# menezesandre/stackrl

Hardware: AMD Instinct MI355X
Metric: env steps/sec (batched Stack-v0) (higher is better)
Workload: dtype f32

## Files before the change

### include/stackrl_qnet.h

```cpp
#ifndef STACKRL_QNET_H_
#define STACKRL_QNET_H_

#include <stdint.h>

#ifdef __cplusplus
extern "C" {
#endif

int srl_xcorr_forward(const float* x_dev, const float* w_dev, float* out_dev, int32_t B, int32_t C, int32_t H,
                      int32_t W, int32_t kh, int32_t kw, void* stream);

int64_t srl_xcorr_mfma_scratch_bytes(int32_t mode, int32_t precision, int32_t B, int32_t C, int32_t H, int32_t kh);
int srl_xcorr_mfma(int32_t mode, int32_t precision, const void* in_dev, int32_t in_f32, const void* kern_dev,
                   int32_t kern_f32, float* out_dev, void* scratch_dev, int64_t scratch_bytes, int32_t B, int32_t C,
                   int32_t H, int32_t kh, void* stream);
const char* srl_xcorr_mfma_last_error(void);

int srl_bias_act(const void* in_dev, void* out_dev, const float* bias_dev, int64_t npix, int32_t C, int32_t out_stride,
                 int32_t out_offset, int32_t nchw_hw, int32_t relu, void* stream);
int srl_bias_act_pool(const void* in_dev, void* skip_dev, void* pooled_dev, const float* bias_dev, int32_t B, int32_t H,
                      int32_t W, int32_t C, int32_t skip_stride, int32_t skip_offset, void* stream);
int srl_bias_act_f32(const float* in_dev, float* out_dev, const float* bias_dev, int64_t npix, int32_t C,
                     int32_t out_stride, int32_t out_offset, int32_t nchw_hw, int32_t relu, void* stream);
int srl_bias_act_pool_f32(const float* in_dev, float* skip_dev, float* pooled_dev, const float* bias_dev, int32_t B,
// ... 57 lines not shown

int srl_baseline_select(const double* values_dev, const uint8_t* mask_dev, int32_t use_goal, int32_t minorder,
                        int64_t* actions_dev, double* neg_values_dev, int32_t B, int32_t OH, void* stream);

const char* srl_qnet_last_error(void);
const char* srl_qnet_build_info(void);

int srl_td_epilogue(const float* q_dev, const float* q_next_online_dev, const float* q_next_target_dev,
                    const int64_t* actions_dev, const float* rewards_dev, const uint8_t* terminal_dev,
                    const float* weights_dev, float gamma, float huber_delta, float reward_scale, int32_t use_double,
                    float prio_eps, int32_t mb, int32_t A, float* loss_dev, float* mean_td_dev, float* td_abs_dev,
                    float* logits_dev, float* grad_q_dev, float* scratch_dev, int32_t* ticket_dev, void* stream);

int srl_adam_step(float* params_dev, const float* grads_dev, float* m_dev, float* v_dev, int64_t n, float* state_dev,
                  float lr, float beta1, float beta2, float eps, void* stream);

int64_t srl_gumbel_topk_scratch_bytes(int64_t n, int32_t k);
int srl_gumbel_topk(const float* logits_dev, const float* u_dev, const float* alpha_dev, int64_t n, int32_t k,
                    int64_t* out_idx_dev, float* out_key_dev, void* scratch_dev, int64_t scratch_bytes, void* stream);

int srl_replay_scatter(const uint8_t* state0_dev, const uint8_t* state1_dev, int64_t bytes0, int64_t bytes1,
                       const float* reward_dev, const uint8_t* terminal_dev, const int64_t* action_dev, int32_t B,
                       int64_t slot, int64_t part_len, uint8_t* mem0_dev, uint8_t* mem1_dev, float* mem_reward_dev,
                       uint8_t* mem_terminal_dev, int64_t* mem_action_dev, float* mem_logits_dev, void* stream);
int srl_replay_gather(const int64_t* idx_dev, int32_t mb, int64_t part_len, int64_t n_steps, int32_t literal_next,
                      int64_t* next_dev, const uint8_t* mem0_dev, const uint8_t* mem1_dev, int64_t bytes0, int64_t bytes1,
                      const float* mem_reward_dev, const uint8_t* mem_terminal_dev, const int64_t* mem_action_dev,
                      const float* mem_logits_dev, const float* alpha_dev, const float* beta_dev,
                      const float* min_logit_dev, uint8_t* state0_dev, uint8_t* state1_dev, uint8_t* next0_dev,
                      uint8_t* next1_dev, int64_t* action_dev, float* reward_dev, uint8_t* terminal_dev,
                      float* weight_dev, void* stream);
int64_t srl_logit_extrema_scratch_bytes(void);
int srl_logit_extrema(const float* logits_dev, int64_t n, float* out_v2_dev, int64_t* out_i2_dev, void* scratch_dev, void* stream);
const char* srl_learner_last_error(void);

int srl_tconv(const float* x_dev, int32_t x_stride, int32_t x_off, const float* wp_dev, const float* bias_dev, float* y_dev,
              int32_t y_stride, int32_t y_off, int32_t B, int32_t H, int32_t W, int32_t cin, int32_t cout, int32_t taps,
              int32_t relu, int32_t d2s, void* stream);
int64_t srl_twrw_scratch_floats(int32_t B, int32_t H, int32_t W, int32_t cin, int32_t cout, int32_t taps);
int srl_twrw(const float* x_dev, int32_t x_stride, int32_t x_off, const float* gz_dev, float* gw_dev, float* scratch_dev,
             int32_t B, int32_t H, int32_t W, int32_t cin, int32_t cout, int32_t taps, int32_t convt,
             const float* bias_partial_dev, int32_t bias_nblk, int32_t bias_C, float* gbias_dev, void* stream);
int64_t srl_tact_bwd_scratch_floats(int64_t npix, int32_t C);
int32_t srl_tact_bwd_blocks(int64_t npix, int32_t C);
int srl_tact_bwd(const float* g_dev, int32_t g_stride, int32_t g_off, const float* y_dev, int32_t y_stride, int32_t y_off,
                 const float* gpool_dev, float* gz_dev, float* gbias_dev, float* scratch_dev, int32_t B, int32_t H, int32_t W,
                 int32_t C, int32_t relu, int32_t s2d, void* stream);
int srl_trepack(const float* flat_dev, float* packed_dev, const int64_t* desc_dev, int32_t nlayers, int64_t total, void* stream);
int srl_thead_fwd(const float* z_dev, const float* pw_dev, const float* pb_dev, const float* v_dev, float* q_dev, int32_t B,
                  int32_t A, void* stream);
int srl_thead_bwd(const float* z_dev, const float* pw_dev, const float* gq_dev, float* gz_dev, float* gv_dev, float* gpw_dev,
                  float* gpb_dev, float* scratch_dev, int32_t n, int32_t A, void* stream);
int srl_tvalue_fwd(const float* x0_dev, const float* W1_dev, const float* b1_dev, const float* W2_dev, const float* b2_dev,
                   float* pooled_dev, float* h_dev, float* v_dev, int32_t B, int32_t P, int32_t C, int32_t U, void* stream);
int srl_tvalue_bwd(const float* gv_dev, const float* h_dev, const float* pooled_dev, const float* W1_dev, const float* W2_dev,
                   const float* gin_dev, float* gx_dev, float* gW1_dev, float* gb1_dev, float* gW2_dev, float* gb2_dev,
                   float* scratch_dev, int32_t n, int32_t P, int32_t C, int32_t U, void* stream);
int srl_tlayout(const float* src_dev, int32_t src_stride, int32_t src_off, float* dst_dev, int32_t B, int32_t HW, int32_t C,
                int32_t to_nhwc, void* stream);
int srl_tcorr_grad(const float* g_dev, int32_t g_stride, float* plain_dev, float* padded_dev, int32_t n, int32_t O, int32_t pad,
                   void* stream);
int srl_tflip(const float* in_dev, float* out_dev, int64_t planes, int32_t hw, void* stream);
int srl_tu8_to_f32(const uint8_t* in_dev, float* out_dev, int64_t n, void* stream);
const char* srl_train_conv_last_error(void);

#ifdef __cplusplus
// ... 4 lines not shown
```

### stackrl_amd/csrc/learner.hip

```cpp
#include <hip/hip_runtime.h>
#include <stdint.h>
#include <math.h>
#include "../../include/stackrl_qnet.h"

namespace {

thread_local char g_err[256] = "";
int fail(const char* m) { snprintf(g_err, sizeof g_err, "%s", m); return 1; }
#define HIPCHK(x) do { hipError_t e_ = (x); if (e_ != hipSuccess) return fail(hipGetErrorString(e_)); } while (0)

__device__ __forceinline__ uint32_t f2o(float f) {
  const uint32_t u = __float_as_uint(f);
  return u ^ ((uint32_t)((int32_t)u >> 31) | 0x80000000u);
}
__device__ __forceinline__ uint64_t vkey(float v, uint32_t idx) { return ((uint64_t)f2o(v) << 32) | (uint32_t)(~idx); }

__device__ __forceinline__ uint64_t wave_max_u64(uint64_t k) {
#pragma unroll
  for (int s = 32; s >= 1; s >>= 1) {
    const uint32_t lo = __shfl_xor((uint32_t)k, s), hi = __shfl_xor((uint32_t)(k >> 32), s);
    const uint64_t o = ((uint64_t)hi << 32) | lo;
    k = o > k ? o : k;
  }
  return k;
}

template <int T>
__device__ __forceinline__ uint64_t block_max_u64(uint64_t k, uint64_t* sh) {
  k = wave_max_u64(k);
  const int w = threadIdx.x >> 6;
  __syncthreads();
  if ((threadIdx.x & 63) == 0) sh[w] = k;
  __syncthreads();
  uint64_t r = sh[0];
#pragma unroll
  for (int i = 1; i < T / 64; ++i) r = sh[i] > r ? sh[i] : r;
// ... 208 lines not shown
__device__ __forceinline__ void ext_take(Ext& a, const Ext& b) {
  if (b.mx > a.mx || (b.mx == a.mx && b.imx < a.imx)) { a.mx = b.mx; a.imx = b.imx; }
  if (b.mn < a.mn || (b.mn == a.mn && b.imn < a.imn)) { a.mn = b.mn; a.imn = b.imn; }
}
__device__ __forceinline__ Ext ext_block(Ext e, Ext* sh) {
  sh[threadIdx.x] = e;
  __syncthreads();
  for (int s = 128; s >= 1; s >>= 1) {
    if ((int)threadIdx.x < s) { Ext a = sh[threadIdx.x]; ext_take(a, sh[threadIdx.x + s]); sh[threadIdx.x] = a; }
    __syncthreads();
  }
  return sh[0];
}
__global__ void __launch_bounds__(256) k_logit_extrema(const float* __restrict__ logits, long long n, Ext* __restrict__ part) {
  __shared__ Ext sh[256];
  Ext e; e.mx = -INFINITY; e.imx = 0x7fffffffffffffffLL; e.mn = INFINITY; e.imn = 0x7fffffffffffffffLL;
  for (long long i = (long long)blockIdx.x * 256 + threadIdx.x; i < n; i += (long long)gridDim.x * 256) {
    const float v = logits[i];
    Ext o; o.mx = v; o.imx = i; o.mn = (v - v == 0.0f) ? v : INFINITY; o.imn = i;
    ext_take(e, o);
  }
  const Ext r = ext_block(e, sh);
  if (threadIdx.x == 0) part[blockIdx.x] = r;
}
__global__ void __launch_bounds__(256) k_logit_extrema_finish(const Ext* __restrict__ part, int nblk, float* __restrict__ out_v,
                                                              long long* __restrict__ out_i) {
  __shared__ Ext sh[256];
  Ext e; e.mx = -INFINITY; e.imx = 0x7fffffffffffffffLL; e.mn = INFINITY; e.imn = 0x7fffffffffffffffLL;
  if ((int)threadIdx.x < nblk) e = part[threadIdx.x];
  const Ext r = ext_block(e, sh);
  if (threadIdx.x == 0) { out_v[0] = r.mx; out_i[0] = r.imx; out_v[1] = r.mn; out_i[1] = r.imn; }
}

}

extern "C" {

const char* srl_learner_last_error(void) { return g_err; }

int srl_td_epilogue(const float* q, const float* qn_online, const float* qn_target, const int64_t* actions,
                    const float* rewards, const uint8_t* terminal, const float* weights, float gamma, float huber_delta,
                    float reward_scale, int32_t use_double, float prio_eps, int32_t mb, int32_t A, float* out_loss,
                    float* out_mtd, float* td_abs, float* logits, float* grad_q, float* scratch, int32_t* ticket,
                    void* stream) {
  if (!q || !qn_target || (use_double && !qn_online) || !actions || !rewards || !terminal || !out_loss || !out_mtd ||
      !td_abs || !logits || !scratch || !ticket || mb < 1 || A < 1)
    return fail("srl_td_epilogue: bad argument");
  hipLaunchKernelGGL((k_td_epilogue<256>), dim3(mb), dim3(256), 0, (hipStream_t)stream, q, qn_online, qn_target, actions,
                     rewards, terminal, weights, gamma, huber_delta, reward_scale, (int)use_double, prio_eps, (int)mb, (int)A,
                     out_loss, out_mtd, td_abs, logits, grad_q, scratch, (int*)ticket);
  HIPCHK(hipGetLastError());
  return 0;
}

int srl_adam_step(float* params, const float* grads, float* m, float* v, int64_t n, float* state, float lr, float beta1,
                  float beta2, float eps, void* stream) {
  if (!params || !grads || !m || !v || !state || n < 1) return fail("srl_adam_step: bad argument");
  if (((uintptr_t)params | (uintptr_t)grads | (uintptr_t)m | (uintptr_t)v) & 15) return fail("srl_adam_step: buffers must be 16-byte aligned");
  hipLaunchKernelGGL(k_adam_tick, dim3(1), dim3(64), 0, (hipStream_t)stream, state, lr, beta1, beta2);
  const int64_t groups = (n >> 2) + 1;
  hipLaunchKernelGGL(k_adam_step, dim3((unsigned)((groups + 255) / 256)), dim3(256), 0, (hipStream_t)stream, params, grads, m,
                     v, n, (const float*)state, beta1, beta2, eps);
  HIPCHK(hipGetLastError());
  return 0;
}

int64_t srl_gumbel_topk_scratch_bytes(int64_t n, int32_t k) {
  if (n < 1 || k < 1) return -1;
  const int64_t G = (n + SRL_TOPK_CHUNK - 1) / SRL_TOPK_CHUNK;
  return G * k * (int64_t)(sizeof(float) + sizeof(int32_t));
}
// ... 28 lines not shown
  return 0;
}

int srl_replay_gather(const int64_t* idx, int32_t mb, int64_t part_len, int64_t n_steps, int32_t literal_next, int64_t* o_next,
                      const uint8_t* m0, const uint8_t* m1, int64_t bytes0,
                      int64_t bytes1, const float* m_reward, const uint8_t* m_terminal, const int64_t* m_action,
                      const float* m_logits, const float* alpha, const float* beta, const float* min_logit, uint8_t* o_s0,
                      uint8_t* o_s1, uint8_t* o_n0, uint8_t* o_n1, int64_t* o_action, float* o_reward, uint8_t* o_terminal,
                      float* o_weight, void* stream) {
  if (!idx || part_len < 1 || n_steps < 1 || !m0 || !m1 || !m_reward || !m_terminal || !m_action || !m_logits || !o_s0 || !o_s1 || !o_n0 || !o_n1 ||
      !o_action || !o_reward || !o_terminal || mb < 1 || (bytes0 & 15) || (bytes1 & 15) || (o_weight && (!alpha || !beta || !min_logit)))
    return fail("srl_replay_gather: bad argument (rows must be multiples of 16 bytes)");
  const int64_t vec = 2 * ((bytes0 + bytes1) >> 4);
  const unsigned gx = (unsigned)((vec + 255) / 256 > 32 ? 32 : (vec + 255) / 256);
  hipLaunchKernelGGL(k_replay_gather, dim3(gx, mb), dim3(256), 0, (hipStream_t)stream, idx, part_len, n_steps, (int)literal_next, o_next, m0, m1, bytes0, bytes1, m_reward,
                     m_terminal, m_action, m_logits, alpha, beta, min_logit, o_s0, o_s1, o_n0, o_n1, o_action, o_reward, o_terminal,
                     o_weight);
  HIPCHK(hipGetLastError());
  return 0;
}

int64_t srl_logit_extrema_scratch_bytes(void) { return 256 * (int64_t)sizeof(Ext); }

int srl_logit_extrema(const float* logits, int64_t n, float* out_v2, int64_t* out_i2, void* scratch, void* stream) {
  if (!logits || n < 1 || !out_v2 || !out_i2 || !scratch) return fail("srl_logit_extrema: bad argument");
  const int nblk = (int)((n + 1023) / 1024 > 256 ? 256 : (n + 1023) / 1024);
  hipStream_t st = (hipStream_t)stream;
  hipLaunchKernelGGL(k_logit_extrema, dim3(nblk), dim3(256), 0, st, logits, (long long)n, (Ext*)scratch);
  hipLaunchKernelGGL(k_logit_extrema_finish, dim3(1), dim3(256), 0, st, (const Ext*)scratch, nblk, out_v2, (long long*)out_i2);
  HIPCHK(hipGetLastError());
  return 0;
}

}
```

### stackrl_amd/dqn.py

```python
import math

import torch
import torch.distributed as dist

from stackrl_amd.memory import ReplayMemory


CAPTURE_MODE = 'thread_local'


class PolynomialDecay(object):

  def __init__(self, initial_learning_rate, decay_steps, end_learning_rate=0.0001, power=1.0):
    self.initial, self.steps, self.end, self.power = float(initial_learning_rate), int(decay_steps), float(end_learning_rate), float(power)

  def __call__(self, step):
    s = min(int(step), self.steps)
    return (self.initial - self.end) * (1 - s / self.steps) ** self.power + self.end


EXPLORATION_MODES = ['epsilon-greedy', 'boltzmann']


def philox4x32_10(counter, key):
# ... 376 lines not shown
      linear = td_abs - quadratic
      loss = 0.5 * quadratic ** 2 + self._huber_delta * linear
    else:
      loss = 0.5 * td_abs ** 2
    if weights is not None:
      loss = loss * weights
    return loss.mean()

  def _draw(self):
    if self._prioritized:
      indexes, weights, (states, actions, rewards, next_states, terminal) = \
        self._replay_memory.sample(self._minibatch_size, get_weights=True)
    else:
      indexes = weights = None
      states, actions, rewards, next_states, terminal = self._replay_memory.sample(self._minibatch_size)
    return (indexes, weights) + tuple(states) + (actions, rewards) + tuple(next_states) + (terminal,)

  def _next_minibatch(self):
    k = self._prefetch
    if not k:
      flat = self._draw()
    else:
      flat = self._peek_minibatch()
      self._advance_fifo()
    return self._split_minibatch(flat)

  def _peek_minibatch(self):
    if self._fifo is None:
      self._fifo = [tuple(None if t is None else t.clone() for t in self._draw()) for _ in range(self._prefetch)]
    return tuple(None if t is None else t.clone() for t in self._fifo[0])

  def _advance_fifo(self):
    k = self._prefetch
    for i in range(k - 1):
      for dst, src in zip(self._fifo[i], self._fifo[i + 1]):
        if dst is not None:
          dst.copy_(src)
    for dst, src in zip(self._fifo[k - 1], self._draw()):
      if dst is not None:
        dst.copy_(src)

  @staticmethod
  def _split_minibatch(flat):
    indexes, weights = flat[0], flat[1]
    ns = (len(flat) - 5) // 2
    states, actions, rewards = flat[2:2 + ns], flat[2 + ns], flat[3 + ns]
    next_states, terminal = flat[4 + ns:4 + 2 * ns], flat[4 + 2 * ns]
    return indexes, weights, (states, actions, rewards, next_states, terminal)

  def _forward_backward(self, peek=False):
    indexes, weights, (states, actions, rewards, next_states, terminal) = \
      self._split_minibatch(self._peek_minibatch()) if peek else self._next_minibatch()
    if not self._bias_compensation:
      weights = None
    self._last_sample_indexes = indexes
    new_logits = None
    if self._fused and not (self._gamma == 0 and not self._n_step):
      from stackrl_amd import qops
      if self._hand is not None:
        mb = int(actions.shape[0])
        self._hand.refresh()
        with torch.no_grad():
          tq = self._hand_t.forward(next_states)
          if self._n_step:
            rewards = (self._gamma_r * rewards).sum(dim=-1)
        if self._double:
          both = tuple(torch.cat([a, b]) for a, b in zip(states, next_states))
          q2 = self._hand.forward(both, save=True)
          q_all, qo = q2[:mb], q2[mb:].detach()
        else:
          q_all, qo = self._hand.forward(states, save=True), None
# ... 232 lines not shown
```

### stackrl_amd/memory.py

```python
import math

import torch


class ReplayMemory(object):
  def __init__(self, state_spec, max_length, alpha=None, beta=None, iters_counter=None, n_steps=None,
               epsilon=1e-3, seed=None, device=None, reference_next_index=True):
    self.device = torch.device(device) if device is not None else torch.device('cpu')
    self._n_parts = int(state_spec[0][0][0])
    max_length -= max_length % self._n_parts
    self._max_length = max_length // self._n_parts
    self._size = max_length
    self._offsets = torch.arange(self._n_parts, dtype=torch.int64, device=self.device) * self._max_length
    if (callable(alpha) or callable(beta)) and iters_counter is None:
      raise ValueError('iters_counter must be provided with a callable alpha/beta')
    self._alpha = alpha if callable(alpha) else float(alpha or 0.)
    self._beta = beta if callable(beta) else float(1. if beta is None else beta)
    self._iters_counter = iters_counter
    self._n_steps = int(n_steps or 1)
    self._n_range = torch.arange(1, self._n_steps + 1, dtype=torch.int64, device=self.device)
    assert self._max_length > self._n_steps
    if epsilon <= 0:
      raise ValueError('epsilon must be greater than 0')
    self.epsilon = float(epsilon)
# ... 56 lines not shown
  def _extrema(self):
    if self._fused and not self.check:
      from stackrl_amd import qops
      (mv, mi), (nv, ni) = qops.logit_extrema(self._logits, self._ws)
      return (mi, mv), (ni, nv)
    return self._argmax_all(), self._argmin_finite()

  def _argmax_all(self):
    v, idx = torch.max(self._logits, dim=0)
    return idx, v

  def _argmin_finite(self):
    finite = torch.isfinite(self._logits)
    if self.check and not bool(finite.any()):
      raise FloatingPointError('No sampleable transition (failed to compute min logit)')
    masked = torch.where(finite, self._logits, torch.full_like(self._logits, math.inf))
    v, idx = torch.min(masked, dim=0)
    return idx, v

  def add(self, state, reward, terminal, action):
    L = self._max_length
    if self._fused:
      from stackrl_amd import qops
      qops.replay_scatter(tuple(u.to(v.dtype) for u, v in zip(state, self._states)), reward, terminal, action,
                          self._insert_index % L, L, self._states, self._rewards, self._terminal, self._actions, self._logits)
    else:
      idx = self._offsets + self._insert_index % L
      for var, upd in zip(self._states, state):
        var.index_copy_(0, idx, upd.to(var.dtype))
      self._rewards.index_copy_(0, idx, reward.to(torch.float32))
      self._terminal.index_copy_(0, idx, terminal.to(torch.bool))
      self._actions.index_copy_(0, idx, action.to(torch.int64))
      self._logits.index_fill_(0, idx, -math.inf)
    if self._insert_index > 0:
      slot = self._insert_index % L
      hit_max = (self._max_logit_index % L) == slot
      hit_min = (self._min_logit_index % L) == slot
      (i, v), (i2, v2) = self._extrema()
      self._max_logit_index.copy_(torch.where(hit_max, i, self._max_logit_index))
      self._max_logit.copy_(torch.where(hit_max, v, self._max_logit))
      if self.check and bool(hit_min):
        self._argmin_finite()
      i, v = i2, v2
      self._min_logit_index.copy_(torch.where(hit_min, i, self._min_logit_index))
      self._min_logit.copy_(torch.where(hit_min, v, self._min_logit))
    back = self._offsets[:, None] + ((self._insert_index - self._n_range) % L)[None, :]
    boundary = self._terminal[back].any(dim=-1)
    val = torch.where(boundary, torch.full((), -math.inf, device=self.device), self._max_logit)
    self._logits.index_copy_(0, back[:, -1], val.to(torch.float32))
    self._insert_index += 1

  def set_terminal(self):
    idx = self._offsets + (self._insert_index - 1) % self._max_length
    self._terminal.index_fill_(0, idx, True)

  def next_indexes(self, indexes, steps):
    L = self._max_length
    if self._reference_next_index:
      return (indexes + steps) % L + indexes // L
    return (indexes % L + steps) % L + (indexes // L) * L

  def refresh_schedules(self):
    self._alpha_t.fill_(self.alpha); self._beta_t.fill_(self.beta)

  def sample(self, minibatch_size, get_weights=False):
    alpha = self._alpha_t if self.tensor_schedules else self.alpha
# ... 13 lines not shown
    if self._n_steps != 1:
      nxt = self.next_indexes(indexes[:, None], self._n_range[None, :])
    rewards = self._rewards[nxt]
    if get_weights:
      beta = self._beta_t if self.tensor_schedules else self.beta
      weights = torch.exp(beta * alpha * (self._min_logit - self._logits[indexes]))
      return indexes, weights, (states, actions, rewards, next_states, terminal)
    return states, actions, rewards, next_states, terminal

  def _sample_fused(self, u, minibatch_size, get_weights):
    from stackrl_amd import qops
    if not self.tensor_schedules:
      self.refresh_schedules()
    indexes, keys = qops.gumbel_topk(self._logits, u, self._alpha_t, minibatch_size, self._ws)
    if self.check and not bool(torch.isfinite(keys).all()):
      raise FloatingPointError('Not enough elements to sample')
    if self._n_steps != 1:
      states = tuple(s[indexes] for s in self._states)
      nxt = self.next_indexes(indexes, self._n_steps)
      batch = (states, self._actions[indexes], self._rewards[self.next_indexes(indexes[:, None], self._n_range[None, :])],
               tuple(s[nxt] for s in self._states), self._terminal[nxt])
      weights = torch.exp(self._beta_t * self._alpha_t * (self._min_logit - self._logits[indexes])) if get_weights else None
    else:
      batch, weights = qops.replay_gather(indexes, self._max_length, 1, self._reference_next_index, self._states, self._rewards,
                                          self._terminal, self._actions, self._logits,
                                          *((self._alpha_t, self._beta_t, self._min_logit) if get_weights else ()))
    if get_weights:
      return indexes, weights, batch
    return batch

  def update_priorities(self, indexes, deltas, logits=None):
    if logits is None:
      logits = torch.log(deltas.to(torch.float32) + self.epsilon)
    self._logits.index_copy_(0, indexes, logits)
    max_logit, amax = torch.max(logits, dim=0); min_logit, amin = torch.min(logits, dim=0)
    imax = indexes.gather(0, amax.view(1))[0]; imin = indexes.gather(0, amin.view(1))[0]
    hit_max = (indexes == self._max_logit_index).any()
    hit_min = (indexes == self._min_logit_index).any()
    (ri, rv), (ri2, rv2) = self._extrema()
    ge = max_logit >= self._max_logit
    self._max_logit_index.copy_(torch.where(ge, imax, torch.where(hit_max, ri, self._max_logit_index)))
    self._max_logit.copy_(torch.where(ge, max_logit, torch.where(hit_max, rv, self._max_logit)))
    ri, rv = ri2, rv2
    le = min_logit <= self._min_logit
    self._min_logit_index.copy_(torch.where(le, imin, torch.where(hit_min, ri, self._min_logit_index)))
    self._min_logit.copy_(torch.where(le, min_logit, torch.where(hit_min, rv, self._min_logit)))
```

### stackrl_amd/metrics.py

```python
import time

import torch


class Timer(object):

  def __init__(self, clock=None):
    if isinstance(clock, str):
      clock = getattr(time, clock)
    if clock is not None and not callable(clock):
      raise TypeError('clock must be None, the name of a function of the time module, or a callable')
    self._clock = clock or time.perf_counter
    self._t0 = None
    self.total, self.n = 0.0, 0

  def reset(self):
    self.total, self.n = 0.0, 0

  def __enter__(self):
    self._t0 = self._clock()
    return self

  def __exit__(self, *exc):
    self.total += self._clock() - self._t0
# ... 38 lines not shown
  def reset(self):
    self._buf.zero_()
    self._index.zero_()

  def __call__(self, *args, **kwargs):
    return self.add(*args, **kwargs)

  def __iadd__(self, other):
    self.add(other)
    return self

  def __lt__(self, other): return bool(self.result < other)
  def __le__(self, other): return bool(self.result <= other)
  def __ge__(self, other): return bool(self.result >= other)
  def __gt__(self, other): return bool(self.result > other)

  def state_dict(self):
    return {'index': self._index.clone(), 'values': self._values.clone()}

  def load_state_dict(self, d):
    self._index.copy_(d['index']); self._values.copy_(d['values'])


class AverageReward(AverageMetric):

  def __init__(self, batch_size, length=100, dtype=torch.float32, device=None):
    super(AverageReward, self).__init__(length=length, dtype=dtype, device=device)
    self._episode_reward = torch.zeros(int(batch_size), dtype=dtype, device=device)

  def add(self, step):
    reward, terminal = step[-2], step[-1]
    dev = self._values.device
    reward = reward.to(device=dev, dtype=self._values.dtype); terminal = terminal.to(device=dev, dtype=torch.bool)
    self._episode_reward += reward
    rank = torch.cumsum(terminal.to(torch.int64), 0) - 1
    k = terminal.sum()
    keep = terminal & (rank >= k - self._length)
    pos = torch.where(keep, (self._index + rank) % self._length, torch.full_like(rank, self._length))
    self._buf.index_copy_(0, pos, self._episode_reward)
    self._buf[self._length] = 0
    self._index += k
    self._episode_reward = torch.where(terminal, torch.zeros_like(self._episode_reward), self._episode_reward)

  def reset(self, full=False):
    super(AverageReward, self).reset()
    if full:
      self._episode_reward.zero_()

  def state_dict(self):
    d = super(AverageReward, self).state_dict()
    d['episode_reward'] = self._episode_reward.clone()
    return d

  def load_state_dict(self, d):
    super(AverageReward, self).load_state_dict(d)
    self._episode_reward.copy_(d['episode_reward'])
```

### stackrl_amd/qops.py

```python
import ctypes

import torch

from stackrl_amd import _bind

_VP, _I32, _I64, _F32, _F64, _INT = ctypes.c_void_p, ctypes.c_int32, ctypes.c_int64, ctypes.c_float, ctypes.c_double, ctypes.c_int
_QNET, _XCORR, _EPI, _CONV, _GEMM, _LEARN, _TRAIN = ('srl_qnet_last_error', 'srl_xcorr_mfma_last_error', 'srl_epilogue_last_error',
                                                     'srl_conv_last_error', 'srl_conv_gemm_last_error', 'srl_learner_last_error',
                                                     'srl_train_conv_last_error')
_SIGS = {
  'srl_xcorr_forward': (_INT, [_VP] * 3 + [_I32] * 6 + [_VP], _QNET),
  'srl_policy_head': (_INT, [_VP] * 3 + [_F32, _VP, _I32, _I32, _VP], _QNET),
  'srl_boltzmann_head': (_INT, [_VP, _VP, _F32, _VP, _I32, _I32, _VP], _QNET),
  'srl_greedy_head': (_INT, [_VP] * 2 + [_I32] * 4 + [_VP] * 4, _QNET),
  'srl_heuristic': (_INT, [_I32] + [_VP] * 4 + [_I32] * 6 + [_F64, _VP], _QNET),
  'srl_baseline_select': (_INT, [_VP, _VP, _I32, _I32, _VP, _VP, _I32, _I32, _VP], _QNET),
  'srl_heuristic_rows': (_INT, [_I32] + [_VP] * 4 + [_I32] * 8 + [_F64, _VP], _QNET),
  'srl_baseline_rows_select': (_INT, [_VP] * 2 + [_I32] * 6 + [_VP] * 4, _QNET),
  'srl_qnet_last_error': (ctypes.c_char_p, [], None),
  'srl_qnet_build_info': (ctypes.c_char_p, [], None),
  'srl_xcorr_mfma_scratch_bytes': (_I64, [_I32] * 6, None),
  'srl_xcorr_mfma': (_INT, [_I32, _I32, _VP, _I32, _VP, _I32, _VP, _VP, _I64] + [_I32] * 4 + [_VP], _XCORR),
  'srl_xcorr_rows': (_INT, [_I32, _VP, _VP, _I32, _VP] + [_I32] * 4 + [_VP], _XCORR),
  'srl_xcorr_mfma_last_error': (ctypes.c_char_p, [], None),
# ... 24 lines not shown
  'srl_conv3x3_gemm_bias_relu': (_INT, [_VP] * 4 + [_I32] * 7 + [_VP], _GEMM),
  'srl_convt2x2_gemm_supported': (_I32, [_I32] * 2, None),
  'srl_convt2x2_gemm_bias_relu': (_INT, [_VP] * 4 + [_I32] * 8 + [_VP], _GEMM),
  'srl_conv_gemm_last_error': (ctypes.c_char_p, [], None),
  'srl_td_epilogue': (_INT, [_VP] * 7 + [_F32, _F32, _F32, _I32, _F32, _I32, _I32] + [_VP] * 8, _LEARN),
  'srl_adam_step': (_INT, [_VP] * 4 + [_I64, _VP] + [_F32] * 4 + [_VP], _LEARN),
  'srl_gumbel_topk_scratch_bytes': (_I64, [_I64, _I32], None),
  'srl_gumbel_topk': (_INT, [_VP] * 3 + [_I64, _I32] + [_VP] * 3 + [_I64, _VP], _LEARN),
  'srl_replay_scatter': (_INT, [_VP, _VP, _I64, _I64, _VP, _VP, _VP, _I32, _I64, _I64] + [_VP] * 7, _LEARN),
  'srl_replay_gather': (_INT, [_VP, _I32, _I64, _I64, _I32, _VP, _VP, _VP, _I64, _I64] + [_VP] * 16, _LEARN),
  'srl_logit_extrema_scratch_bytes': (_I64, [], None),
  'srl_logit_extrema': (_INT, [_VP, _I64] + [_VP] * 4, _LEARN),
  'srl_learner_last_error': (ctypes.c_char_p, [], None),
  'srl_tconv': (_INT, [_VP, _I32, _I32, _VP, _VP, _VP] + [_I32] * 10 + [_VP], _TRAIN),
  'srl_twrw_scratch_floats': (_I64, [_I32] * 6, None),
  'srl_twrw': (_INT, [_VP, _I32, _I32, _VP, _VP, _VP] + [_I32] * 7 + [_VP, _I32, _I32, _VP, _VP], _TRAIN),
  'srl_tact_bwd_scratch_floats': (_I64, [_I64, _I32], None),
  'srl_tact_bwd_blocks': (_I32, [_I64, _I32], None),
  'srl_tact_bwd': (_INT, [_VP, _I32, _I32, _VP, _I32, _I32] + [_VP] * 4 + [_I32] * 6 + [_VP], _TRAIN),
  'srl_trepack': (_INT, [_VP, _VP, _VP, _I32, _I64, _VP], _TRAIN),
  'srl_thead_fwd': (_INT, [_VP] * 5 + [_I32, _I32, _VP], _TRAIN),
  'srl_thead_bwd': (_INT, [_VP] * 8 + [_I32, _I32, _VP], _TRAIN),
  'srl_tvalue_fwd': (_INT, [_VP] * 8 + [_I32] * 4 + [_VP], _TRAIN),
  'srl_tvalue_bwd': (_INT, [_VP] * 12 + [_I32] * 4 + [_VP], _TRAIN),
  'srl_tlayout': (_INT, [_VP, _I32, _I32, _VP] + [_I32] * 4 + [_VP], _TRAIN),
  'srl_tcorr_grad': (_INT, [_VP, _I32, _VP, _VP, _I32, _I32, _I32, _VP], _TRAIN),
  'srl_tflip': (_INT, [_VP, _VP, _I64, _I32, _VP], _TRAIN),
  'srl_tu8_to_f32': (_INT, [_VP, _VP, _I64, _VP], _TRAIN),
  'srl_train_conv_last_error': (ctypes.c_char_p, [], None),
}


load, call = _bind.binding('qnet', _SIGS)
_stream = _bind.stream


_SCRATCH = {}
MFMA_SHAPES = ((128, 32), (64, 16))
BF16, BF16X3 = 0, 1


def _xcorr_mfma(mode, precision, a, k, B, C, H, kh):
  if not a.is_cuda:
    raise RuntimeError('the MFMA cross-correlation needs a HIP device (no CPU fallback)')
  if precision == BF16X3:
    a = a.float(); k = k.float()
  a = a.contiguous(); k = k.contiguous()
  for t in (a, k):
    if t.dtype not in (torch.float32, torch.bfloat16):
      raise TypeError('xcorr operands must be float32 or bfloat16')
  L = load()
  need = L.srl_xcorr_mfma_scratch_bytes(mode, precision, B, C, H, kh)
  if need < 0:
    raise RuntimeError('MFMA cross-correlation: unsupported shape (H=%d, kh=%d)' % (H, kh))
  key = (a.device.index, torch.cuda.current_stream(a.device).cuda_stream)
  scratch = _SCRATCH.get(key)
  if scratch is None or scratch.numel() < need:
    scratch = torch.empty(need, dtype=torch.uint8, device=a.device)
    _SCRATCH[key] = scratch
  O = H - kh + 1
  shape = {0: (B, 1, O, O), 1: (B, C, H, H), 2: (B, C, kh, kh)}[mode]
  out = torch.empty(shape, dtype=torch.float32, device=a.device)
  call('srl_xcorr_mfma', a, mode, precision, a, int(a.dtype == torch.float32), k, int(k.dtype == torch.float32), out, scratch,
       scratch.numel(), B, C, H, kh)
  return out

# ... 705 lines not shown
  term = terminal.contiguous().view(torch.uint8)
  act = actions.contiguous(); rew = rewards.contiguous().float()
  wts = weights.contiguous().float() if weights is not None else None
  call('srl_td_epilogue', q, q, qo, qt, act, rew, term, wts, float(gamma), -1.0 if huber_delta is None else float(huber_delta),
       float(reward_scale or 0.0), int(bool(double)), float(prio_eps), mb, A, out, out[1:], td_abs, logits, grad_q, ws['scratch'], ws['ticket'])
  return out[0], out[1], td_abs, logits, grad_q


def adam_step(params, grads, m, v, state, lr, beta1, beta2, eps):
  call('srl_adam_step', params, params, grads, m, v, params.numel(), state, float(lr), float(beta1), float(beta2), float(eps))


def gumbel_topk(logits, u, alpha_t, k, ws):
  n = logits.numel()
  need = load().srl_gumbel_topk_scratch_bytes(n, k)
  if ws.get('topk_n') != (n, k):
    ws['topk_n'] = (n, k)
    ws['topk_scratch'] = torch.empty(need, dtype=torch.uint8, device=logits.device)
  idx = torch.empty(k, dtype=torch.int64, device=logits.device)
  key = torch.empty(k, dtype=torch.float32, device=logits.device)
  call('srl_gumbel_topk', logits, logits, u, alpha_t, n, k, idx, key, ws['topk_scratch'], need)
  return idx, key


def replay_scatter(state, reward, terminal, action, slot, part_len, mem_states, mem_reward, mem_terminal, mem_action, mem_logits):
  s0, s1 = (t.contiguous() for t in state)
  B = s0.shape[0]
  b0, b1 = s0[0].numel() * s0.element_size(), s1[0].numel() * s1.element_size()
  r = reward.contiguous().float(); t = terminal.contiguous().to(torch.bool).view(torch.uint8); a = action.contiguous().to(torch.int64)
  call('srl_replay_scatter', s0, s0, s1, b0, b1, r, t, a, B, int(slot), int(part_len), mem_states[0], mem_states[1], mem_reward,
       mem_terminal, mem_action, mem_logits)


def logit_extrema(logits, ws):
  dev = logits.device
  if 'ext' not in ws:
    ws['ext'] = torch.empty(int(load().srl_logit_extrema_scratch_bytes()), dtype=torch.uint8, device=dev)
  v = torch.empty(2, dtype=torch.float32, device=dev)
  i = torch.empty(2, dtype=torch.int64, device=dev)
  call('srl_logit_extrema', logits, logits, logits.numel(), v, i, ws['ext'])
  return (v[0], i[0]), (v[1], i[1])


def replay_gather(idx, part_len, n_steps, literal_next, mem_states, mem_reward, mem_terminal, mem_action, mem_logits,
                  alpha_t=None, beta_t=None, min_logit=None):
  mb = idx.numel()
  m0, m1 = mem_states
  dev = m0.device
  b0, b1 = m0[0].numel() * m0.element_size(), m1[0].numel() * m1.element_size()
  s0 = torch.empty((mb,) + tuple(m0.shape[1:]), dtype=m0.dtype, device=dev); n0 = torch.empty_like(s0)
  s1 = torch.empty((mb,) + tuple(m1.shape[1:]), dtype=m1.dtype, device=dev); n1 = torch.empty_like(s1)
  act = torch.empty(mb, dtype=torch.int64, device=dev)
  rew = torch.empty(mb, dtype=torch.float32, device=dev)
  term = torch.empty(mb, dtype=torch.bool, device=dev)
  w = torch.empty(mb, dtype=torch.float32, device=dev) if alpha_t is not None else None
  call('srl_replay_gather', m0, idx, mb, int(part_len), int(n_steps), int(bool(literal_next)), None, m0, m1, b0, b1, mem_reward,
       mem_terminal, mem_action, mem_logits, alpha_t, beta_t, min_logit, s0, s1, n0, n1, act, rew, term, w)
  return ((s0, s1), act, rew, (n0, n1), term), w
```

Measured before the change: 100,400.

## Fuse collect-loop bookkeeping (reward tracking, replay priority, FIFO shift) into HIP kernels

Adds HIP kernels that replace several chains of small torch ops in the collection loop: episode-reward tracking with a block scan, replay max/min-logit tracking on insert, a single multi-tensor FIFO shift for prefetched minibatches, and priority updates with a fused scatter and extrema recompute. The aim is to cut kernel-launch and Python dispatch overhead per environment step. In exchange it adds single-block kernels that serialise work for large batches, caps batch and tensor counts, and builds a host pointer table on every FIFO advance.

After: 100,200. About the same (-0.2%).

```diff
diff --git a/include/stackrl_collect.h b/include/stackrl_collect.h
--- /dev/null
+++ b/include/stackrl_collect.h
@@ -0,0 +1,23 @@
+#ifndef STACKRL_COLLECT_H
+#define STACKRL_COLLECT_H
+#include <stdint.h>
+#ifdef __cplusplus
+extern "C" {
+#endif
+
+int srlc_reward_track(const float* reward_dev, const uint8_t* terminal_dev, int32_t B, float* episode_reward_dev, float* buf_dev,
+                     int64_t length, int64_t* index_dev, void* stream);
+int srlc_replay_track(const float* ext_v2_dev, const int64_t* ext_i2_dev, int64_t slot, int64_t back, int64_t part_len, int32_t B,
+                     const uint8_t* mem_terminal_dev, float* mem_logits_dev, float* max_logit_dev, int64_t* max_index_dev,
+                     float* min_logit_dev, int64_t* min_index_dev, void* stream);
+int srlc_fifo_advance(const int64_t* table_host, int32_t n_tensors, int32_t n_slots, void* stream);
+int64_t srlc_priority_update_scratch_bytes(void);
+int srlc_priority_update(const int64_t* idx_dev, const float* new_logits_dev, int32_t mb, float* mem_logits_dev, int64_t n,
+                        float* max_logit_dev, int64_t* max_index_dev, float* min_logit_dev, int64_t* min_index_dev,
+                        void* scratch_dev, void* stream);
+const char* srlc_last_error(void);
+
+#ifdef __cplusplus
+}
+#endif
+#endif
diff --git a/include/stackrl_qnet.h b/include/stackrl_qnet.h
--- a/include/stackrl_qnet.h
+++ b/include/stackrl_qnet.h
@@ -113,6 +113,7 @@
                       float* weight_dev, void* stream);
 int64_t srl_logit_extrema_scratch_bytes(void);
 int srl_logit_extrema(const float* logits_dev, int64_t n, float* out_v2_dev, int64_t* out_i2_dev, void* scratch_dev, void* stream);
+
 const char* srl_learner_last_error(void);
 
 int srl_tconv(const float* x_dev, int32_t x_stride, int32_t x_off, const float* wp_dev, const float* bias_dev, float* y_dev,
diff --git a/stackrl_amd/csrc/learner.hip b/stackrl_amd/csrc/learner.hip
--- a/stackrl_amd/csrc/learner.hip
+++ b/stackrl_amd/csrc/learner.hip
@@ -1,7 +1,9 @@
 #include <hip/hip_runtime.h>
 #include <stdint.h>
 #include <math.h>
+#include <string.h>
 #include "../../include/stackrl_qnet.h"
+#include "../../include/stackrl_collect.h"
 
 namespace {
 
@@ -276,11 +278,138 @@
   if (threadIdx.x == 0) { out_v[0] = r.mx; out_i[0] = r.imx; out_v[1] = r.mn; out_i[1] = r.imn; }
 }
 
+
+template <int T>
+__device__ __forceinline__ int block_excl_scan(int v, int* sh, int* total) {
+  const int lane = threadIdx.x & 63, w = threadIdx.x >> 6;
+  int inc = v;
+#pragma unroll
+  for (int s = 1; s < 64; s <<= 1) { const int o = __shfl_up(inc, s); if (lane >= s) inc += o; }
+  __syncthreads();
+  if (lane == 63) sh[w] = inc;
+  __syncthreads();
+  int base = 0, tot = 0;
+#pragma unroll
+  for (int i = 0; i < T / 64; ++i) { const int c = sh[i]; if (i < w) base += c; tot += c; }
+  *total = tot;
+  return base + inc - v;
+}
+
+#define SRL_REWARD_T 1024
+#define SRL_REWARD_MAX_B 16384
+__global__ void __launch_bounds__(SRL_REWARD_T) k_reward_track(const float* __restrict__ reward, const uint8_t* __restrict__ terminal,
+    int B, float* __restrict__ episode_reward, float* __restrict__ buf, long long length, long long* __restrict__ index) {
+  __shared__ int sh[SRL_REWARD_T / 64];
+  const int per = (B + SRL_REWARD_T - 1) / SRL_REWARD_T;
+  const int b0 = min(B, (int)threadIdx.x * per), b1 = min(B, b0 + per);
+  const long long idx0 = index[0];
+  int cnt = 0;
+  for (int b = b0; b < b1; ++b) cnt += terminal[b] != 0;
+  int k;
+  long long rank = block_excl_scan<SRL_REWARD_T>(cnt, sh, &k);
+  for (int b = b0; b < b1; ++b) {
+    float e = episode_reward[b] + reward[b];
+    if (terminal[b]) {
+      if (rank >= (long long)k - length) buf[(idx0 + rank) % length] = e;
+      ++rank;
+      e = 0.0f;
+    }
+    episode_reward[b] = e;
+  }
+  if (threadIdx.x == 0) { buf[length] = 0.0f; index[0] = idx0 + k; }
+}
+
+__global__ void __launch_bounds__(256) k_replay_track(const float* __restrict__ ext_v, const long long* __restrict__ ext_i,
+    long long slot, long long back, long long part_len, int B, const uint8_t* __restrict__ m_terminal, float* __restrict__ m_logits,
+    float* __restrict__ max_logit, long long* __restrict__ max_index, float* __restrict__ min_logit, long long* __restrict__ min_index) {
+  __shared__ float s_max;
+  if (threadIdx.x == 0) {
+    float mx = max_logit[0];
+    if (ext_v) {
+      if (max_index[0] % part_len == slot) { max_index[0] = ext_i[0]; mx = ext_v[0]; max_logit[0] = mx; }
+      if (min_index[0] % part_len == slot) { min_index[0] = ext_i[1]; min_logit[0] = ext_v[1]; }
+    }
+    s_max = mx;
+  }
+  __syncthreads();
+  const float mx = s_max;
+  for (int b = threadIdx.x; b < B; b += 256) {
+    const long long row = (long long)b * part_len + back;
+    m_logits[row] = m_terminal[row] ? -INFINITY : mx;
+  }
+}
+
+#define SRL_FIFO_TENSORS 9
+#define SRL_FIFO_SLOTS 8
+struct FifoArgs {
+  uint8_t* p[SRL_FIFO_TENSORS][SRL_FIFO_SLOTS + 1];
+  long long bytes[SRL_FIFO_TENSORS];
+  int vec[SRL_FIFO_TENSORS];
+  int k;
+};
+template <typename V>
+__device__ __forceinline__ void fifo_shift(uint8_t* const* p, int k, long long j) {
+  V v[SRL_FIFO_SLOTS];
+#pragma unroll
+  for (int s = 0; s < SRL_FIFO_SLOTS; ++s) if (s < k) v[s] = ((const V*)p[s + 1])[j];
+#pragma unroll
+  for (int s = 0; s < SRL_FIFO_SLOTS; ++s) if (s < k) ((V*)p[s])[j] = v[s];
+}
+__global__ void __launch_bounds__(256) k_fifo_advance(const FifoArgs a) {
+  const int t = blockIdx.y;
+  uint8_t* p[SRL_FIFO_SLOTS + 1];
+#pragma unroll
+  for (int s = 0; s <= SRL_FIFO_SLOTS; ++s) p[s] = a.p[t][s];
+  const long long nv = a.vec[t] ? a.bytes[t] >> 4 : 0, tail = a.bytes[t] - (nv << 4);
+  for (long long i = (long long)blockIdx.x * 256 + threadIdx.x; i < nv + tail; i += (long long)gridDim.x * 256) {
+    if (i < nv) fifo_shift<uint4>(p, a.k, i);
+    else fifo_shift<uint8_t>(p, a.k, (nv << 4) + (i - nv));
+  }
+}
+
+struct PrioMb { long long i[2]; float v[2]; int hit[2]; };
+__global__ void __launch_bounds__(256) k_priority_scatter(const long long* __restrict__ idx, const float* __restrict__ new_logits,
+    int mb, float* __restrict__ m_logits, long long n, const long long* __restrict__ max_index, const long long* __restrict__ min_index,
+    PrioMb* __restrict__ out) {
+  __shared__ Ext sh[256];
+  const long long tmax = max_index[0], tmin = min_index[0];
+  Ext e; e.mx = -INFINITY; e.imx = 0x7fffffffffffffffLL; e.mn = INFINITY; e.imn = 0x7fffffffffffffffLL;
+  int hmax = 0, hmin = 0;
+  for (int j = threadIdx.x; j < mb; j += 256) {
+    const long long i = idx[j];
+    const float v = new_logits[j];
+    if ((unsigned long long)i < (unsigned long long)n) m_logits[i] = v;
+    Ext o; o.mx = v; o.imx = j; o.mn = v; o.imn = j;
+    ext_take(e, o);
+    hmax |= i == tmax; hmin |= i == tmin;
+  }
+  const Ext r = ext_block(e, sh);
+  hmax = __syncthreads_or(hmax); hmin = __syncthreads_or(hmin);
+  if (threadIdx.x == 0) {
+    out->v[0] = r.mx; out->i[0] = idx[r.imx < mb ? r.imx : 0]; out->v[1] = r.mn; out->i[1] = idx[r.imn < mb ? r.imn : 0];
+    out->hit[0] = hmax != 0; out->hit[1] = hmin != 0;
+  }
+}
+__global__ void __launch_bounds__(256) k_priority_finish(const Ext* __restrict__ part, int nblk, const PrioMb* __restrict__ mbx,
+    float* __restrict__ max_logit, long long* __restrict__ max_index, float* __restrict__ min_logit, long long* __restrict__ min_index) {
+  __shared__ Ext sh[256];
+  Ext e; e.mx = -INFINITY; e.imx = 0x7fffffffffffffffLL; e.mn = INFINITY; e.imn = 0x7fffffffffffffffLL;
+  if ((int)threadIdx.x < nblk) e = part[threadIdx.x];
+  const Ext r = ext_block(e, sh);
+  if (threadIdx.x == 0) {
+    if (mbx->v[0] >= max_logit[0]) { max_index[0] = mbx->i[0]; max_logit[0] = mbx->v[0]; }
+    else if (mbx->hit[0]) { max_index[0] = r.imx; max_logit[0] = r.mx; }
+    if (mbx->v[1] <= min_logit[0]) { min_index[0] = mbx->i[1]; min_logit[0] = mbx->v[1]; }
+    else if (mbx->hit[1]) { min_index[0] = r.imn; min_logit[0] = r.mn; }
+  }
+}
+
 }
 
 extern "C" {
 
 const char* srl_learner_last_error(void) { return g_err; }
+const char* srlc_last_error(void) { return g_err; }
 
 int srl_td_epilogue(const float* q, const float* qn_online, const float* qn_target, const int64_t* actions,
                     const float* rewards, const uint8_t* terminal, const float* weights, float gamma, float huber_delta,
@@ -375,4 +504,76 @@
   return 0;
 }
 
-}
+int srlc_reward_track(const float* reward, const uint8_t* terminal, int32_t B, float* episode_reward, float* buf, int64_t length,
+                     int64_t* index, void* stream) {
+  if (!reward || !terminal || !episode_reward || !buf || !index || B < 1 || B > SRL_REWARD_MAX_B || length < 1)
+    return fail("srlc_reward_track: bad argument (1 <= B <= 16384, length >= 1)");
+  hipLaunchKernelGGL(k_reward_track, dim3(1), dim3(SRL_REWARD_T), 0, (hipStream_t)stream, reward, terminal, (int)B, episode_reward,
+                     buf, (long long)length, (long long*)index);
+  HIPCHK(hipGetLastError());
+  return 0;
+}
+
+int srlc_replay_track(const float* ext_v2, const int64_t* ext_i2, int64_t slot, int64_t back, int64_t part_len, int32_t B,
+                     const uint8_t* m_terminal, float* m_logits, float* max_logit, int64_t* max_index, float* min_logit,
+                     int64_t* min_index, void* stream) {
+  if (!m_terminal || !m_logits || !max_logit || !max_index || !min_logit || !min_index || B < 1 || part_len < 1 || slot < 0 ||
+      slot >= part_len || back < 0 || back >= part_len || (!ext_v2) != (!ext_i2))
+    return fail("srlc_replay_track: bad argument");
+  hipLaunchKernelGGL(k_replay_track, dim3(1), dim3(256), 0, (hipStream_t)stream, ext_v2, (const long long*)ext_i2, (long long)slot,
+                     (long long)back, (long long)part_len, (int)B, m_terminal, m_logits, max_logit, (long long*)max_index, min_logit,
+                     (long long*)min_index);
+  HIPCHK(hipGetLastError());
+  return 0;
+}
+
+int srlc_fifo_advance(const int64_t* table_host, int32_t n_tensors, int32_t n_slots, void* stream) {
+  if (!table_host || n_tensors < 1 || n_tensors > SRL_FIFO_TENSORS || n_slots < 1 || n_slots > SRL_FIFO_SLOTS)
+    return fail("srlc_fifo_advance: bad argument (at most 9 tensors, 8 slots)");
+  FifoArgs a;
+  memset(&a, 0, sizeof a);
+  a.k = (int)n_slots;
+  long long most = 0;
+  for (int t = 0; t < n_tensors; ++t) {
+    const int64_t* row = table_host + (size_t)t * (n_slots + 2);
+    uintptr_t all = 0;
+    for (int s = 0; s <= n_slots; ++s) {
+      if (!row[s]) return fail("srlc_fifo_advance: null pointer in the table");
+      for (int r = 0; r < s; ++r)
+        if (row[r] == row[s]) return fail("srlc_fifo_advance: two slots of a tensor share their address");
+      a.p[t][s] = (uint8_t*)(uintptr_t)row[s];
+      all |= (uintptr_t)row[s];
+    }
+    if (row[n_slots + 1] < 1) return fail("srlc_fifo_advance: a tensor of no bytes");
+    a.bytes[t] = (long long)row[n_slots + 1];
+    a.vec[t] = (all & 15) == 0;
+    const long long work = a.vec[t] ? (a.bytes[t] >> 4) + (a.bytes[t] & 15) : a.bytes[t];
+    most = work > most ? work : most;
+  }
+  const unsigned gx = (unsigned)((most + 255) / 256 > 64 ? 64 : (most + 255) / 256);
+  hipLaunchKernelGGL(k_fifo_advance, dim3(gx, n_tensors), dim3(256), 0, (hipStream_t)stream, a);
+  HIPCHK(hipGetLastError());
+  return 0;
+}
+
+int64_t srlc_priority_update_scratch_bytes(void) { return 256 * (int64_t)sizeof(Ext) + (int64_t)sizeof(PrioMb); }
+
+int srlc_priority_update(const int64_t* idx, const float* new_logits, int32_t mb, float* m_logits, int64_t n, float* max_logit,
+                        int64_t* max_index, float* min_logit, int64_t* min_index, void* scratch, void* stream) {
+  if (!idx || !new_logits || mb < 1 || mb > 1024 || !m_logits || n < 1 || !max_logit || !max_index || !min_logit || !min_index ||
+      !scratch || ((uintptr_t)scratch & 15))
+    return fail("srlc_priority_update: bad argument (1 <= minibatch <= 1024, 16-byte aligned scratch)");
+  Ext* part = (Ext*)scratch;
+  PrioMb* mbx = (PrioMb*)(part + 256);
+  const int nblk = (int)((n + 1023) / 1024 > 256 ? 256 : (n + 1023) / 1024);
+  hipStream_t st = (hipStream_t)stream;
+  hipLaunchKernelGGL(k_priority_scatter, dim3(1), dim3(256), 0, st, (const long long*)idx, new_logits, (int)mb, m_logits, (long long)n,
+                     (const long long*)max_index, (const long long*)min_index, mbx);
+  hipLaunchKernelGGL(k_logit_extrema, dim3(nblk), dim3(256), 0, st, (const float*)m_logits, (long long)n, part);
+  hipLaunchKernelGGL(k_priority_finish, dim3(1), dim3(256), 0, st, (const Ext*)part, nblk, (const PrioMb*)mbx, max_logit,
+                     (long long*)max_index, min_logit, (long long*)min_index);
+  HIPCHK(hipGetLastError());
+  return 0;
+}
+
+}
diff --git a/stackrl_amd/dqn.py b/stackrl_amd/dqn.py
--- a/stackrl_amd/dqn.py
+++ b/stackrl_amd/dqn.py
@@ -432,11 +432,17 @@
 
   def _advance_fifo(self):
     k = self._prefetch
+    fresh = None
+    if self.device.type == 'cuda':
+      from stackrl_amd import qops
+      fresh = self._draw()
+      if qops.fifo_supported(self._fifo, fresh):
+        return qops.fifo_advance(self._fifo, fresh)
     for i in range(k - 1):
       for dst, src in zip(self._fifo[i], self._fifo[i + 1]):
         if dst is not None:
           dst.copy_(src)
-    for dst, src in zip(self._fifo[k - 1], self._draw()):
+    for dst, src in zip(self._fifo[k - 1], fresh if fresh is not None else self._draw()):
       if dst is not None:
         dst.copy_(src)
 
diff --git a/stackrl_amd/memory.py b/stackrl_amd/memory.py
--- a/stackrl_amd/memory.py
+++ b/stackrl_amd/memory.py
@@ -112,6 +112,12 @@
       self._terminal.index_copy_(0, idx, terminal.to(torch.bool))
       self._actions.index_copy_(0, idx, action.to(torch.int64))
       self._logits.index_fill_(0, idx, -math.inf)
+    if self._fused and not self.check and self._n_steps == 1:
+      ext = qops.logit_extrema(self._logits, self._ws, raw=True) if self._insert_index > 0 else None
+      qops.replay_track(ext, self._insert_index % L, (self._insert_index - 1) % L, L, self._n_parts, self._terminal.view(torch.uint8),
+                        self._logits, self._max_logit, self._max_logit_index, self._min_logit, self._min_logit_index)
+      self._insert_index += 1
+      return
     if self._insert_index > 0:
       slot = self._insert_index % L
       hit_max = (self._max_logit_index % L) == slot
@@ -191,6 +197,11 @@
   def update_priorities(self, indexes, deltas, logits=None):
     if logits is None:
       logits = torch.log(deltas.to(torch.float32) + self.epsilon)
+    if self._fused and not self.check:
+      from stackrl_amd import qops
+      qops.priority_update(indexes, logits.to(torch.float32), self._logits, self._max_logit, self._max_logit_index, self._min_logit,
+                           self._min_logit_index, self._ws)
+      return
     self._logits.index_copy_(0, indexes, logits)
     max_logit, amax = torch.max(logits, dim=0); min_logit, amin = torch.min(logits, dim=0)
     imax = indexes.gather(0, amax.view(1))[0]; imin = indexes.gather(0, amin.view(1))[0]
diff --git a/stackrl_amd/metrics.py b/stackrl_amd/metrics.py
--- a/stackrl_amd/metrics.py
+++ b/stackrl_amd/metrics.py
@@ -94,6 +94,10 @@
     reward, terminal = step[-2], step[-1]
     dev = self._values.device
     reward = reward.to(device=dev, dtype=self._values.dtype); terminal = terminal.to(device=dev, dtype=torch.bool)
+    if dev.type == 'cuda' and self._buf.dtype == torch.float32:
+      from stackrl_amd import qops
+      if self._episode_reward.numel() <= qops.REWARD_TRACK_MAX_B:
+        return qops.reward_track(reward, terminal, self._episode_reward, self._buf, self._length, self._index)
     self._episode_reward += reward
     rank = torch.cumsum(terminal.to(torch.int64), 0) - 1
     k = terminal.sum()
diff --git a/stackrl_amd/qops.py b/stackrl_amd/qops.py
--- a/stackrl_amd/qops.py
+++ b/stackrl_amd/qops.py
@@ -80,6 +80,17 @@
 
 
 load, call = _bind.binding('qnet', _SIGS)
+
+_COLLECT = 'srlc_last_error'
+_COLLECT_SIGS = {
+  'srlc_reward_track': (_INT, [_VP, _VP, _I32, _VP, _VP, _I64, _VP, _VP], _COLLECT),
+  'srlc_replay_track': (_INT, [_VP, _VP, _I64, _I64, _I64, _I32] + [_VP] * 7, _COLLECT),
+  'srlc_fifo_advance': (_INT, [_VP, _I32, _I32, _VP], _COLLECT),
+  'srlc_priority_update_scratch_bytes': (_I64, [], None),
+  'srlc_priority_update': (_INT, [_VP, _VP, _I32, _VP, _I64] + [_VP] * 6, _COLLECT),
+  'srlc_last_error': (ctypes.c_char_p, [], None),
+}
+load_collect, call_collect = _bind.binding('qnet', _COLLECT_SIGS)
 _stream = _bind.stream
 
 
@@ -851,14 +862,64 @@
        mem_terminal, mem_action, mem_logits)
 
 
-def logit_extrema(logits, ws):
+def logit_extrema(logits, ws, raw=False):
   dev = logits.device
   if 'ext' not in ws:
     ws['ext'] = torch.empty(int(load().srl_logit_extrema_scratch_bytes()), dtype=torch.uint8, device=dev)
   v = torch.empty(2, dtype=torch.float32, device=dev)
   i = torch.empty(2, dtype=torch.int64, device=dev)
   call('srl_logit_extrema', logits, logits, logits.numel(), v, i, ws['ext'])
+  if raw:
+    return v, i
   return (v[0], i[0]), (v[1], i[1])
+
+
+REWARD_TRACK_MAX_B = 16384
+FIFO_MAX_TENSORS, FIFO_MAX_SLOTS = 9, 8
+
+
+def reward_track(reward, terminal, episode_reward, buf, length, index):
+  B = episode_reward.numel()
+  if reward.dtype != torch.float32 or terminal.dtype != torch.bool or reward.numel() != B or terminal.numel() != B:
+    raise ValueError('reward_track: reward float32 [{0}] and terminal bool [{0}] expected'.format(B))
+  if buf.numel() != int(length) + 1 or not (episode_reward.is_contiguous() and buf.is_contiguous()):
+    raise ValueError('reward_track: buf must be contiguous and hold length + 1 values')
+  call_collect('srlc_reward_track', buf, reward.contiguous(), terminal.contiguous().view(torch.uint8), B, episode_reward, buf, int(length), index)
+
+
+def replay_track(ext, slot, back, part_len, B, mem_terminal, mem_logits, max_logit, max_index, min_logit, min_index):
+  v, i = ext if ext is not None else (None, None)
+  call_collect('srlc_replay_track', mem_logits, v, i, int(slot), int(back), int(part_len), int(B), mem_terminal, mem_logits, max_logit, max_index,
+       min_logit, min_index)
+
+
+def fifo_supported(slots, fresh):
+  live = [j for j, t in enumerate(fresh) if t is not None]
+  if not live or len(live) > FIFO_MAX_TENSORS or not 1 <= len(slots) <= FIFO_MAX_SLOTS:
+    return False
+  for j in live:
+    for t in [s[j] for s in slots]:
+      if t is None or not t.is_cuda or t.dtype != fresh[j].dtype or t.shape != fresh[j].shape or not t.is_contiguous() or t.numel() == 0:
+        return False
+    if not (fresh[j].is_cuda and fresh[j].is_contiguous()):
+      return False
+  return True
+
+
+def fifo_advance(slots, fresh):
+  live = [j for j, t in enumerate(fresh) if t is not None]
+  table = torch.tensor([[s[j].data_ptr() for s in slots] + [fresh[j].data_ptr(), fresh[j].numel() * fresh[j].element_size()] for j in live],
+                       dtype=torch.int64)
+  call_collect('srlc_fifo_advance', fresh[live[0]], table, len(live), len(slots))
+
+
+def priority_update(indexes, new_logits, mem_logits, max_logit, max_index, min_logit, min_index, ws):
+  if indexes.dtype != torch.int64 or new_logits.dtype != torch.float32 or indexes.numel() != new_logits.numel():
+    raise ValueError('priority_update: indexes int64 [mb] and logits float32 [mb] expected')
+  if 'prio' not in ws:
+    ws['prio'] = torch.empty(int(load_collect().srlc_priority_update_scratch_bytes()), dtype=torch.uint8, device=mem_logits.device)
+  call_collect('srlc_priority_update', mem_logits, indexes.contiguous(), new_logits.contiguous(), indexes.numel(), mem_logits, mem_logits.numel(),
+       max_logit, max_index, min_logit, min_index, ws['prio'])
 
 
 def replay_gather(idx, part_len, n_steps, literal_next, mem_states, mem_reward, mem_terminal, mem_action, mem_logits,
```
